# PixArt-alpha/PixArt-sigma

Measured on AMD Instinct MI355X. Metric: denoising steps/sec (fwd+bwd) PixArt-Sigma-XL/2 1024px bs16 @1/2/4/8 GPU, higher is better.
Workload: dtype fp16; 1 GPU; PixArt-Sigma-XL/2 1024px training step (fwd+bwd+clip+AdamW), batch 16/GPU, L=300 text tokens, DP=1 RCCL all-reduce; model=PixArtMS_XL_2, global_batch=16, seq_len=4096, parallelism=dp1, grad_checkpoint=False, optimizer=adamw, text_lens=all 300

## Files before the change

### pixart_sigma_amd/csrc/gemm.hip

```cpp
#include <atomic>
#include "common.h"
#include "gemm_params.h"
#include "../../include/pixart_hip.h"
#include <cstdio>
#include <cstdlib>
#include <cstring>

namespace {
using namespace pxa;

constexpr int BM = 128, BN = 128, BK = 64;
constexpr int KC_BYTES = 128 * BK * 2;
constexpr int RC_STRIDE = (128 + 32) * 2;
constexpr int RC_BYTES = BK * RC_STRIDE;


template <bool KC>
__device__ __forceinline__ void g2r(const bf16_t* __restrict__ X, int ld, int r0, int R, int k0, int kend, uint4 (&reg)[4], int tid) {
#pragma unroll
  for (int i = 0; i < 4; i++) {
    const bf16_t* src;
    bool ok;
    if (KC) {
      int c = tid & 7, row = (tid >> 3) + 32 * i;
// ... 566 lines not shown
    return frag_p<true, 256, 32>(lds, rbase, ks, lane);
  } else {
    const int gg = lane >> 4, tt = lane & 15, hi2 = gg >> 1;
    const int kr = ks * 16 + 8 * hi2 + (tt >> 2), col = rbase + 16 * (gg & 1) + (tt & 3) * 4;
    const int blk = col >> 5, inblk = (col & 31) * 2;
    const char* p0 = lds + (kr << (rows_log2 + 1)) + ((blk ^ (kr & 3)) << 6) + inblk;
    const char* p1 = lds + ((kr + 4) << (rows_log2 + 1)) + ((blk ^ ((kr + 4) & 3)) << 6) + inblk;
    return concat_tr(lds_tr_read(p0), lds_tr_read(p1));
  }
}

__device__ __forceinline__ bf16x8 frag16_kc(const char* lds, int rbase, int lane) {
  const int row = rbase + (lane & 15);
  return *reinterpret_cast<const bf16x8*>(lds + row * 64 + (((lane >> 4) ^ kc_swz<true>(row)) << 4));
}
template <bool KC>
__device__ __forceinline__ bf16x8 frag16(const char* lds, int rbase, int lane, int rows_log2) {
  if constexpr (KC) {
    return frag16_kc(lds, rbase, lane);
  } else {
    const int gg = lane >> 4, tt = lane & 15;
    const int kr = 8 * gg + (tt >> 2), col = rbase + (tt & 3) * 4;
    const int blk = col >> 5, inblk = ((col & 31) * 2) ^ ((gg & 1) << 5);
    const char* p0 = lds + (kr << (rows_log2 + 1)) + ((blk ^ (kr & 3)) << 6) + inblk;
    const char* p1 = lds + ((kr + 4) << (rows_log2 + 1)) + ((blk ^ ((kr + 4) & 3)) << 6) + inblk;
    return concat_tr(lds_tr_read(p0), lds_tr_read(p1));
  }
}

#ifndef GEMM_TRACE
#define GEMM_TRACE 0
#endif
#if GEMM_TRACE
__device__ unsigned long long g_trace[12][8];
#define PXA_TR(k) do { if (blockIdx.x == 8 && tid == 0 && tr_i < 12) g_trace[tr_i][k] = __builtin_readcyclecounter(); } while (0)
#else
#define PXA_TR(k) do {} while (0)
#endif
__device__ unsigned g_sched[64][16];
__device__ unsigned g_sched_word[64][512];

template <int LAYOUT, int EPI, int RM, bool SEG = false>
__global__ __launch_bounds__(512) void gemm_pers_kernel(GemmParams p) {
  constexpr bool A_KC = (LAYOUT != 2), B_KC = (LAYOUT == 0);
  constexpr int NW = 8, TM = 4, TN = 2, BKT = 32, H1 = 2;
  constexpr bool PH16 = GEMM_PHASE16 < 0 ? (LAYOUT != 0) : (GEMM_PHASE16 != 0);
  constexpr bool M16 = ((GEMM_M16 >> LAYOUT) & 1) && !(GEMM_ABL & 4);
  constexpr int UNIT = 40960;
  extern __shared__ __attribute__((aligned(16))) char smem[];
  const int tid = threadIdx.x, lane = tid & 63, wave = __builtin_amdgcn_readfirstlane(tid >> 6), wm = wave >> 2, wn = wave & 3, hi = lane >> 5;
  const bool late = wave >= NW / 2;
  char* stg = smem + 3 * UNIT + wave * 4096;
  const int mt = (p.M + 255) / 256, ntf = p.N / 256, remn = p.N - ntf * 256;
  constexpr bool PAIR = (RM == 1), HALF = (RM == 2);
  const bool remcol = RM != 0 && remn > 0 && remn <= 128;
  const int ntp = remcol ? ntf : (p.N + 255) / 256;
  const int rem_pg = remcol ? (PAIR ? 4 : 8) : 0;
  const int per_group = 8 * ntp + rem_pg, tiles = mt * ntp + (remcol ? (PAIR ? (mt + 1) / 2 : mt) : 0), T = tiles * p.split;
  auto units_of = [&](int z) { return (min(p.K, (z + 1) * p.k_per_split) - z * p.k_per_split) / BKT; };

  int m0a = 0, m0b = 0, n0 = 0, z_ = 0;
  bool vt = false;
  const int xq = T / 8, xr = T % 8;
  auto xs = [&](int x) { return x * xq + min(x, xr); };
  auto xc = [&](int x) { return xq + (x < xr ? 1 : 0); };
  auto locate_g = [&](int Lg) {
    z_ = Lg / tiles;
    const int t = Lg - z_ * tiles;
    const int g = t / per_group, in_g = t - g * per_group, first_m = g * 8, gsz = min(mt - first_m, 8), nfull = gsz * ntp;
    if (in_g < nfull) { vt = false; m0a = (first_m + in_g % gsz) * 256; m0b = m0a; n0 = (in_g / gsz) * 256; }
    else if (PAIR) { vt = true; m0a = (first_m + 2 * (in_g - nfull)) * 256; m0b = m0a + 256; n0 = ntf * 256; }
    else if (HALF) { vt = true; m0a = (first_m + (in_g - nfull)) * 256; m0b = m0a; n0 = ntf * 256; }
  };
  const bool rev = LAYOUT != 2 && p.desc != 0;
  auto pos_of = [&](int x, int i) { return xs(x) + (rev ? xc(x) - 1 - i : i); };
  auto locate = [&](int L) { locate_g(pos_of(L % 8, L / 8)); };
  const bool DYN = p.sched_slot >= 0;
  const int myx = blockIdx.x % 8;
  unsigned* sched = g_sched[p.sched_slot & 63];
  unsigned* sched_lds = reinterpret_cast<unsigned*>(smem + 32768);
  unsigned* sched_glb = &g_sched_word[p.sched_slot & 63][blockIdx.x & 511];
  auto publish = [&](int v) {
    if (PAIR) { if (lane == 0) __hip_atomic_store(sched_glb, (unsigned)v, __ATOMIC_RELAXED, __HIP_MEMORY_SCOPE_AGENT); wait_vmcnt<0>(); }
    else { if (lane == 0) sched_lds[0] = (unsigned)v; asm volatile("s_waitcnt lgkmcnt(0)" ::: "memory"); }
  };
  auto receive = [&]() -> int {
    const unsigned v = PAIR ? __hip_atomic_load(sched_glb, __ATOMIC_RELAXED, __HIP_MEMORY_SCOPE_AGENT) : sched_lds[0];
    return __builtin_amdgcn_readfirstlane((int)v);
  };
  unsigned pend = 0u;
  int nxt = -1;
  auto fetch_issue = [&]() {
    if (wave == 0 && lane == 0) {
      unsigned* cur = &sched[myx];
      const unsigned one = 1u;
      asm volatile("global_atomic_add %0, %1, %2, off sc0" : "=v"(pend) : "v"(cur), "v"(one) : "memory");
    }
  };
  auto fetch_resolve = [&]() -> int {
    int res = -1;
    asm volatile("" : "+v"(pend));
    if (lane == 0) {
      if ((int)pend < xc(myx)) res = pos_of(myx, (int)pend);
      else
        for (int k = 1; k < 8 && res < 0; k++) {
          const int x2 = (myx + k) & 7;
          const unsigned i2 = atomicAdd(&sched[x2], 1u);
          if ((int)i2 < xc(x2)) res = pos_of(x2, (int)i2);
        }
    }
    return __builtin_amdgcn_readfirstlane(res);
  };
  int L = blockIdx.x;
#if GEMM_STAGGER
  if (LAYOUT != 2 && ((blockIdx.x >> 3) & 1)) {
    const unsigned long long t0 = __builtin_amdgcn_s_memrealtime();
    while (__builtin_amdgcn_s_memrealtime() - t0 < (unsigned long long)GEMM_STAGGER) __builtin_amdgcn_s_sleep(32);
  }
#endif
  if (DYN) {
    fetch_issue();
    wait_vmcnt<0>();
// ... 3 lines not shown
    __syncthreads();
    if (first < 0) {
      if (wave == 0 && lane == 0 && atomicAdd(&sched[8], 1u) == gridDim.x - 1)
        for (int k = 0; k < 9; k++) sched[k] = 0u;
      return;
    }
    locate_g(first);
    fetch_issue();
  } else {
    locate(L);
  }
  int nk = units_of(z_), nk_pf = nk;
  const bf16_t* pp[5];
  long st[5];
  int dof[5];
  const long stepA = A_KC ? BKT : (long)BKT * p.lda, stepB = B_KC ? BKT : (long)BKT * p.ldb;
  int s_lo = 0, s_hi = 0;
  bool vt_pf = false;
  int dma_count = 0;
  auto piece = [&](int i, int slot) {
    dma_count++;
    lds_dma16(pp[i], smem + slot * UNIT + dof[i]);
#if !(GEMM_ABL & 1)
    pp[i] += st[i];
#endif
  };
  int seg_left0 = 0, seg_left1 = 0;
  int tap_kx0 = 0, tap_ky0 = 0, tap_half0 = 0, tap_kx1 = 0, tap_ky1 = 0, tap_half1 = 0;
#define PXA_SEG_ADVANCE(seg_left, tap_kx, tap_ky, tap_half, pa, pb)                                                          \
  do {                                                                                                                       \
    if (p.k_tap) {                                             \
      if (tap_half) {                                                                                                        \
        long adj;                                                                                                            \
        if (tap_kx < 2) { adj = p.k_tap - 64; tap_kx++; }                                                                    \
        else if (tap_ky < 2) { adj = p.tap_s - 2L * p.k_tap - 64; tap_kx = 0; tap_ky++; }                                    \
        else { adj = -2L * p.tap_s - 2L * p.k_tap; tap_kx = 0; tap_ky = 0; }                                                 \
        pa += adj; pb += adj;                                                                                                \
      }                                                                                                                      \
      tap_half ^= 1;                                                                                                         \
    } else {                                                                                                                 \
      seg_left -= BKT;                                                                                                       \
      if (seg_left == 0) { pa += p.seg_jump; pb += p.seg_jump; seg_left = p.k_seg; }                                         \
    }                                                                                                                        \
  } while (0)
  auto issue_lo = [&]() __attribute__((always_inline)) {
#pragma unroll
    for (int i = 0; i < H1; i++) piece(i, s_lo);
    if (SEG) PXA_SEG_ADVANCE(seg_left0, tap_kx0, tap_ky0, tap_half0, pp[0], pp[1]);
    s_lo = (s_lo + 1) & 3;
  };
  auto issue_hi = [&]() __attribute__((always_inline)) {
    piece(2, s_hi);
    if (!(HALF && vt_pf)) piece(3, s_hi);
    if (PAIR && vt_pf) piece(4, s_hi);
    if (SEG && PAIR) { if (vt_pf) PXA_SEG_ADVANCE(seg_left1, tap_kx1, tap_ky1, tap_half1, pp[2], pp[3]); }
    s_hi = (s_hi + 1) & 3;
  };
#undef PXA_SEG_ADVANCE
  auto prefetch = [&]() __attribute__((always_inline)) {
    vt_pf = (RM != 0) && vt;
    const long k0 = (long)z_ * p.k_per_split;
    const bool vq = PAIR && vt, hq = HALF && vt;
    const int rla = vq ? 9 : 8, rlb = (vq || hq) ? 7 : 8;
    const int ln = opaque<LAYOUT == 1 || (EPI >= 2 && EPI != 7) || (GEMM_EPI_EARLY && RM == 2)>(lane);
#pragma unroll
    for (int i = 0; i < 5; i++) {
      const int id = wave + NW * i;
      const bool is_a = vq ? (i < 4) : (i < 2);
      const int pid = is_a ? id : (vq ? id - 32 : id - 16);
      if (vq || (hq ? i < 3 : i < 4)) {
        if (is_a) pp[i] = piece_ptr_rt<A_KC, M16>(p.A, p.lda, m0a, m0b, p.M, pid * 64 + ln, rla) + (A_KC ? k0 : k0 * p.lda);
        else pp[i] = piece_ptr_rt<B_KC, M16>(p.B, p.ldb, n0, n0, p.N, pid * 64 + ln, rlb) + (B_KC ? k0 : k0 * p.ldb);
      }
      st[i] = is_a ? stepA : stepB;
      dof[i] = (is_a ? 0 : (vq ? 32768 : 16384)) + pid * 1024;
    }
    s_lo = s_hi = 0;
    dma_count = 0;
    if (SEG) { seg_left0 = seg_left1 = p.k_seg; tap_kx0 = tap_kx1 = tap_ky0 = tap_ky1 = tap_half0 = tap_half1 = 0; }
    issue_lo(); issue_hi(); issue_lo(); issue_hi();
    if (nk_pf > 2) { issue_lo(); if (PH16) issue_hi(); }
  };
  prefetch();
  int tr_i = 0; (void)tr_i;
  int prev_stores = 0;

  while (true) {
    f32x16 acc[TM][TN];
    f32x4 acc4[2 * TM][2 * TN];
#pragma unroll
    for (int i = 0; i < TM; i++)
#pragma unroll
      for (int j = 0; j < TN; j++)
#pragma unroll
        for (int g = 0; g < 16; g++) acc[i][j][g] = 0.f;
#pragma unroll
    for (int i = 0; i < 2 * TM; i++)
#pragma unroll
      for (int j = 0; j < 2 * TN; j++) acc4[i][j] = f32x4{0.f, 0.f, 0.f, 0.f};
#if GEMM_ABL & 4
    f32x4 a4[TM][TN][4];
#pragma unroll
    for (int i = 0; i < TM; i++)
#pragma unroll
      for (int j = 0; j < TN; j++)
#pragma unroll
        for (int q = 0; q < 4; q++) a4[i][j][q] = f32x4{0.f, 0.f, 0.f, 0.f};
#endif
    const bool vtc = PAIR && vt, hfc = HALF && vt;
    const int a_rb = hfc ? (wave >> 1) * 64 : (vtc ? (wn >> 1) * 256 : 0) + wm * 128, b_rb = (vtc || hfc) ? (wn & 1) * 64 : wn * 64;
    const int rla = vtc ? 9 : 8, rlb = (vtc || hfc) ? 7 : 8, boff = vtc ? 32768 : 16384;
    const int mw = hfc ? m0a + a_rb : ((vtc && (wn >> 1)) ? m0b : m0a) + wm * 128, nw = n0 + b_rb;
    const int tm_eff = hfc ? 2 : TM;
    const int zw = z_;
    PXA_TR(0);
    if (GEMM_STORE_OVERLAP && LAYOUT != 2 && EPI != 3) {
      if (prev_stores == 40) wait_vmcnt<40>();
      else if (prev_stores == 36) wait_vmcnt<36>();
      else if (prev_stores == 32) wait_vmcnt<32>();
      else if (prev_stores == 28) wait_vmcnt<28>();
      else if (prev_stores == 24) wait_vmcnt<24>();
      else if (prev_stores == 20) wait_vmcnt<20>();
      else if (prev_stores == 16) wait_vmcnt<16>();
      else if (prev_stores == 12) wait_vmcnt<12>();
      else if (prev_stores == 8) wait_vmcnt<8>();
      else wait_vmcnt<0>();
    } else {
      wait_vmcnt<0>();
    }
    if (DYN && wave == 0) {
      publish(fetch_resolve());
    }
    __builtin_amdgcn_s_barrier();
    if (DYN) nxt = receive();
    if (late) __builtin_amdgcn_s_barrier();
    PXA_TR(1);
    constexpr bool EARLY = GEMM_EPI_EARLY && M16 && LAYOUT != 2;
    constexpr bool AUXA = EARLY && (EPI == 2 || EPI == 4 || EPI == 6) && !(GEMM_ABL & 16);
    typedef unsigned u32x2 __attribute__((ext_vector_type(2)));
    u32x2 axa[2][2][4];
    f32x4 bq[2 * TN];
    const bool has_bias = EARLY && p.bias != nullptr;
    auto bias_issue = [&]() {
      const int R4b = lane >> 4;
#pragma unroll
      for (int jn = 0; jn < 2 * TN; jn++) {
        const float* src = p.bias + min(nw + jn * 16 + 4 * R4b, p.N - 4);
        asm volatile("global_load_dwordx4 %0, %1, off" : "=v"(bq[jn]) : "v"(src) : "memory");
      }
    };
    auto aux_issue = [&](int i, u32x2 (&dst)[2][4]) {
      const int R4a = lane >> 4, c16a = lane & 15;
#pragma unroll
      for (int mh = 0; mh < 2; mh++)
#pragma unroll
        for (int jn = 0; jn < 4; jn++) {
          const int m = min(mw + i * 32 + 16 * mh + c16a, p.M - 1), n = min(nw + jn * 16 + 4 * R4a, p.N - 4);
          const bf16_t* src = p.aux + (size_t)m * p.ldaux + n;
          asm volatile("global_load_dwordx2 %0, %1, off" : "=v"(dst[mh][jn]) : "v"(src) : "memory");
        }
    };
    auto unit16 = [&](int t, auto rem_c, auto th_c) {
// ... 131 lines not shown
#pragma unroll
    for (int i = 0; i < TM; i++)
#pragma unroll
      for (int j = 0; j < TN; j++)
#pragma unroll
        for (int g = 0; g < 16; g++) acc[i][j][g] = a4[i][j][g >> 2][g & 3];
#endif
    PXA_TR(2);
    if constexpr (LAYOUT != 2) {
      if (has_bias) bias_issue();
      if constexpr (AUXA) { aux_issue(0, axa[0]); aux_issue(1, axa[1]); }
    }
    if (!late) __builtin_amdgcn_s_barrier();
    PXA_TR(3);

    bool more = false;
    int pf_ops = 0;
    auto hand_over = [&]() {
      if (DYN) {
        more = nxt >= 0;
        if (more) {
          locate_g(nxt);
          nk_pf = units_of(z_);
          prefetch();
          fetch_issue();
        }
      } else {
        L += gridDim.x;
        more = L < T;
        if (more) {
          locate(L);
          nk_pf = units_of(z_);
          prefetch();
        }
      }
      if (more) pf_ops = dma_count;
    };
    const int le = opaque<LAYOUT == 1 || (EPI >= 2 && EPI != 7) || (GEMM_EPI_EARLY && RM == 2)>(lane);
    const int srow = le & 31;
    if constexpr (LAYOUT == 2) {
      hand_over();
      PXA_TR(4);
#pragma unroll
      for (int i = 0; i < TM; i++)
#pragma unroll
        for (int j = 0; j < TN; j++) {
          if constexpr (M16) {
#pragma unroll
            for (int mh = 0; mh < 2; mh++)
#pragma unroll
              for (int nh = 0; nh < 2; nh++) {
                const f32x4 a = acc4[2 * i + mh][2 * j + nh];
                const int row = 16 * mh + (lane & 15);
                *reinterpret_cast<float4*>(stg + row * 128 + (((4 * nh + (lane >> 4)) ^ (row & 7)) << 4)) = make_float4(a[0], a[1], a[2], a[3]);
              }
          } else {
#pragma unroll
          for (int q = 0; q < 4; q++)
            *reinterpret_cast<float4*>(stg + srow * 128 + (((q * 2 + hi) ^ (srow & 7)) << 4)) =
                make_float4(acc[i][j][q * 4], acc[i][j][q * 4 + 1], acc[i][j][q * 4 + 2], acc[i][j][q * 4 + 3]);
          }
          __builtin_amdgcn_s_waitcnt(0xc07f);
#pragma unroll
          for (int t4 = 0; t4 < 4; t4++) {
            const int row = t4 * 8 + (lane >> 3), ch = lane & 7;
            float4 v = *reinterpret_cast<const float4*>(stg + row * 128 + ((ch ^ (row & 7)) << 4));
            const int mm = mw + i * 32 + row, nn = nw + j * 32 + ch * 4;
            if (mm < p.M && nn < p.N) {
              if (p.accumulate == 3) {
                *reinterpret_cast<float4*>(p.slab + ((size_t)zw * p.M + mm) * p.N + nn) = v;
              } else {
                float* dst = p.outf + (size_t)mm * p.ldf + nn;
                if (p.accumulate) { const float4 o = *reinterpret_cast<const float4*>(dst); v.x += o.x; v.y += o.y; v.z += o.z; v.w += o.w; }
                *reinterpret_cast<float4*>(dst) = v;
              }
            }
          }
          __builtin_amdgcn_s_waitcnt(0xc07f);
        }
      nk = nk_pf;
      if (!more) break;
      continue;
    }
    const int act = (EPI == 0 || EPI == 5) ? 0 : EPI == 1 ? 3 : EPI == 2 ? 4 : (EPI == 4 || EPI == 6) ? 5 : EPI == 7 ? 1 : p.act;
    constexpr bool want_st = (EPI == 5 || EPI == 6);
    const bool dual = EPI == 1 || (EPI == 3 && ((p.act == 1 && p.out2 != nullptr) || p.act == 3));
    const bool want_cs = !(GEMM_ABL & 8) && (EPI == 2 || (EPI == 3 && p.colsum != nullptr));
    auto bias_apply = [&]() {
      asm volatile("" : "+v"(bq[0]), "+v"(bq[1]), "+v"(bq[2]), "+v"(bq[3]));
#pragma unroll
      for (int jn = 0; jn < 2 * TN; jn++)
#pragma unroll
        for (int mt = 0; mt < 2 * TM; mt++) acc4[mt][jn] += bq[jn];
    };
    auto bias_add = [&]() {
      const int R4b = le >> 4;
      if constexpr (M16) {
#pragma unroll
        for (int jn = 0; jn < 2 * TN; jn++) {
          const int n = nw + jn * 16 + 4 * R4b;
          const float4 b4 = (p.bias && n < p.N) ? *reinterpret_cast<const float4*>(p.bias + n) : make_float4(0.f, 0.f, 0.f, 0.f);
#pragma unroll
          for (int mt = 0; mt < 2 * TM; mt++) { acc4[mt][jn][0] += b4.x; acc4[mt][jn][1] += b4.y; acc4[mt][jn][2] += b4.z; acc4[mt][jn][3] += b4.w; }
        }
      } else {
#pragma unroll
        for (int j = 0; j < TN; j++)
#pragma unroll
          for (int q = 0; q < 4; q++) {
            const int n = nw + j * 32 + 8 * q + 4 * hi;
            const float4 b4 = (p.bias && n < p.N) ? *reinterpret_cast<const float4*>(p.bias + n) : make_float4(0.f, 0.f, 0.f, 0.f);
#pragma unroll
            for (int i = 0; i < TM; i++) { acc[i][j][q * 4] += b4.x; acc[i][j][q * 4 + 1] += b4.y; acc[i][j][q * 4 + 2] += b4.z; acc[i][j][q * 4 + 3] += b4.w; }
          }
      }
    };
    auto wait_allow = [&](int allowed) {
      if (allowed >= 28) wait_vmcnt<28>();
      else if (allowed >= 26) wait_vmcnt<26>();
      else if (allowed >= 24) wait_vmcnt<24>();
// ... 180 lines not shown
        }
      }
      static_assert(!(PAIR && (EPI == 2 || EPI == 3)), "column sums in a paired instance: guard their atomics with mw < p.M as the statistics are");
      if (want_cs) {
#pragma unroll
        for (int e = 0; e < 8; e++) {
          float v = cs[e];
          if (LPR <= 4) v += __shfl_xor(v, 4);
          v += __shfl_xor(v, 8); v += __shfl_xor(v, 16); v += __shfl_xor(v, 32);
          const int n = nw + j0 * 32 + (lane % LPR) * 8 + e;
          if (lane < LPR && n < p.N) atomicAdd(p.colsum + (size_t)((mw >> 7) % PXA_COLSUM_SLOTS) * p.colsum_stride + n, v);
        }
      }
      if (want_st && mw < p.M) {
        float* dst = p.gn_part + ((size_t)((mw >> 7) % PXA_COLSUM_SLOTS) * p.gn_B + st_img) * (p.N / 4) * 2;
#pragma unroll
        for (int h = 0; h < 2; h++) {
          float v = cs[h], u = sq[h];
          if (LPR <= 4) { v += __shfl_xor(v, 4); u += __shfl_xor(u, 4); }
          v += __shfl_xor(v, 8); v += __shfl_xor(v, 16); v += __shfl_xor(v, 32);
          u += __shfl_xor(u, 8); u += __shfl_xor(u, 16); u += __shfl_xor(u, 32);
          const int n = nw + j0 * 32 + (lane % LPR) * 8 + 4 * h;
          if (lane < LPR && n < p.N) { atomicAdd(dst + (n >> 2) * 2, v); atomicAdd(dst + (n >> 2) * 2 + 1, u); }
        }
      }
    };
    if (GEMM_ABL & 2) {
      float sacc = 0.f;
#pragma unroll
      for (int i = 0; i < TM; i++)
#pragma unroll
        for (int j = 0; j < TN; j++) sacc += acc[i][j][0] + acc[i][j][7] + acc[i][j][15];
      if (sacc == 123.456f) p.out[lane] = (bf16_t)sacc;
    } else {
#pragma unroll
      for (int j0 = 0; j0 + 1 < TN; j0 += 2) emit(j0, IntC<2>{});
      if constexpr (TN % 2 == 1) emit(TN - 1, IntC<1>{});
    }
    PXA_TR(5);
#if GEMM_TRACE
    tr_i++;
#endif
    {
      const bool interior = mw + tm_eff * 32 <= p.M && nw + 64 <= p.N;
      prev_stores = (interior && p.out && !(want_st && p.up_rp)) ? tm_eff * 4 * ((dual && !(GEMM_ABL & 32)) ? 2 : 1) + (want_st ? 4 : 0) + (want_cs ? 8 : 0) + ((AUXA && tm_eff > 2) ? 16 : 0) : 0;
    }
    nk = nk_pf;
    if (!more) break;
  }
  if (DYN && wave == 0 && lane == 0 && atomicAdd(&sched[8], 1u) == gridDim.x - 1)
    for (int k = 0; k < 9; k++) sched[k] = 0u;
}

struct GemmKnobs { bool no_staged, no_pers, no_half, seg_half; int tile; bool ascending, no_glds; };
GemmKnobs read_gemm_knobs() {
  static const bool no_staged = getenv("PXA_GEMM_NO_STAGED_EPILOGUE") != nullptr;
  static const bool no_pers = getenv("PXA_GEMM_NO_PERSISTENT") != nullptr;
  static const bool no_half = getenv("PXA_GEMM_NO_HALF_ITEMS") != nullptr;
  static const bool seg_half = getenv("PXA_GEMM_SEG_HALF") != nullptr;
  static const int tile = [] { const char* f = getenv("PXA_GEMM_TILE"); return f ? atoi(f) * (strstr(f, "x128") ? -1 : 1) : 0; }();
  static const bool ascending = getenv("PXA_GEMM_ASCENDING") != nullptr;
  return GemmKnobs{no_staged, no_pers, no_half, seg_half, tile, ascending, getenv("PXA_GEMM_NO_GLDS") != nullptr};
}
int dynamic_items_env() { return getenv("PXA_GEMM_STATIC") ? 0 : getenv("PXA_GEMM_DYNAMIC") ? 1 : -1; }
std::atomic<int> g_dynamic_items{-1}; std::atomic<unsigned> g_launch_seq{0};
bool dynamic_items() {
  int expect = -1;
  if (g_dynamic_items.load(std::memory_order_relaxed) < 0) g_dynamic_items.compare_exchange_strong(expect, dynamic_items_env() == 1 ? 1 : 0);
  return g_dynamic_items.load(std::memory_order_relaxed) != 0;
}
bool pers_halfcol(int N) { return N % 256 > 0 && N % 256 <= 128; }
int pers_tiles(int M, int N, int rm) {
  const int mt = (M + 255) / 256, ntf = N / 256;
  if (rm == 2 && pers_halfcol(N)) return mt * ntf + mt;
  const bool pairing = rm == 1 && pers_halfcol(N);
  return mt * (pairing ? ntf : (N + 255) / 256) + (pairing ? (mt + 1) / 2 : 0);
}
void cost_model(int M, int N, int K, int& split, int& tile) {
  struct Cfg { int tile, bm, bn, slots; double rate; };
  const Cfg cfgs[2] = {{128, 128, 128, 512, 760e12}, {256, 256, 256, 256, 1050e12}};
  double best = 1e30;
  for (const Cfg& c : cfgs) {
    if (c.tile == 256 && (M < 256 || N < 256)) continue;
    const long tiles = c.tile == 256 ? pers_tiles(M, N, 1) : (long)((M + c.bm - 1) / c.bm) * ((N + c.bn - 1) / c.bn);
    for (int sp = 1; sp <= 16; sp++) {
      const int kp = ((K + sp - 1) / sp + BK - 1) / BK * BK;
      if ((long)kp * (sp - 1) >= K) continue;
      const long rounds = (tiles * sp + c.slots - 1) / c.slots;
      const double t = rounds * (double)kp * c.bm * c.bn * 2.0 / (c.rate / c.slots) + (sp > 1 ? 2.0 * sp * M * N * 4.0 / 3.5e12 + 4e-6 : 0.0);
      if (t < best) { best = t; split = sp; tile = c.tile; }
    }
  }
}
int fill_gemm(const pxa_gemm_args* a, const GemmKnobs& k, GemmParams& p, int& tile) {
  PXA_CHECK(a && a->A && a->B, "pxa_gemm: null operand");
  PXA_CHECK(a->layout >= 0 && a->layout <= 2, "pxa_gemm: bad layout %d", a->layout);
  PXA_CHECK(a->M > 0 && a->N > 0 && a->K > 0, "pxa_gemm: bad shape %d %d %d", a->M, a->N, a->K);
  PXA_CHECK(a->N % 8 == 0, "pxa_gemm: N=%d must be a multiple of 8", a->N);
  PXA_CHECK(a->lda % 8 == 0 && a->ldb % 8 == 0, "pxa_gemm: lda/ldb must be multiples of 8 (16-byte rows)");
  if (a->layout != 2) PXA_CHECK(a->K % 8 == 0, "pxa_gemm: K=%d must be a multiple of 8 for k-contiguous A", a->K);
  if (a->layout == 2) PXA_CHECK(a->M % 8 == 0, "pxa_gemm: M=%d must be a multiple of 8 for layout TN", a->M);
  PXA_CHECK(a->out_bf16 || a->out_f32, "pxa_gemm: no output");
  if (a->out_bf16 || a->out2_bf16) PXA_CHECK(a->ld_out % 4 == 0, "pxa_gemm: ld_out must be a multiple of 4");
  if (a->out_f32) PXA_CHECK(a->ld_f32 % 4 == 0, "pxa_gemm: ld_f32 must be a multiple of 4");
  PXA_CHECK(a->act >= 0 && a->act <= 5, "pxa_gemm: bad act %d", a->act);
  if (a->act == 2 || a->act == 4 || a->act == 5) PXA_CHECK(a->aux && a->ldaux % 4 == 0, "pxa_gemm: act=%d needs aux", a->act);
  if (a->act == 3) PXA_CHECK(a->out_bf16 && a->out2_bf16, "pxa_gemm: act=3 needs both bf16 outputs");
  if (a->colsum) PXA_CHECK(a->out_bf16 && !a->out_f32, "pxa_gemm: colsum needs a bf16 output");
  int split = a->split_k < 1 ? 1 : a->split_k;
  if (split > 1) PXA_CHECK(a->out_f32 && a->accumulate && !a->out_bf16 && a->act == 0 && !a->bias, "pxa_gemm: split_k>1 needs fp32 atomic accumulate output only");
  p.A = (const bf16_t*)a->A; p.B = (const bf16_t*)a->B; p.lda = a->lda; p.ldb = a->ldb; p.M = a->M; p.N = a->N; p.K = a->K;
  p.bias = a->bias; p.aux = (const bf16_t*)a->aux; p.ldaux = a->ldaux; p.out = (bf16_t*)a->out_bf16; p.out2 = (bf16_t*)a->out2_bf16; p.ldo = a->ld_out;
  p.outf = a->out_f32; p.ldf = a->ld_f32; p.act = a->act; p.accumulate = a->accumulate; tile = 0;
  p.desc = (a->items_descending && !k.ascending) ? 1 : 0;
  p.k_seg = a->k_seg; p.seg_jump = a->k_seg ? a->a_seg_stride - a->k_seg : 0; p.k_tap = a->k_seg ? a->k_tap : 0; p.tap_s = a->a_seg_stride;
  if (a->k_seg && a->k_tap) PXA_CHECK(a->k_tap % BK == 0 && a->k_seg == 3 * a->k_tap && a->K == 3 * a->k_seg, "pxa_gemm: k_tap=%d needs k_seg = 3 k_tap, K = 9 k_tap, k_tap a multiple of %d", a->k_tap, BK);
  if (a->k_seg) {
    PXA_CHECK(a->layout == 0 && split == 1 && !a->colsum, "pxa_gemm: k_seg needs layout NT, no split-K, no colsum");
    PXA_CHECK(a->k_seg > 0 && a->k_seg % BK == 0 && a->K % a->k_seg == 0 && a->a_seg_stride % 8 == 0, "pxa_gemm: k_seg=%d must be a multiple of %d dividing K=%d (segment stride a multiple of 8)", a->k_seg, BK, a->K);
  }
  if (a->split_k == 0 && a->out_f32 && a->accumulate && !a->out_bf16 && a->act == 0 && !a->bias && a->K % BK == 0) cost_model(a->M, a->N, a->K, split, tile);
  p.k_per_split = ((a->K + split - 1) / split + BK - 1) / BK * BK;
  split = p.split = (a->K + p.k_per_split - 1) / p.k_per_split; p.tile_hint = tile; p.sched_slot = -1; p.slab = nullptr;
  p.colsum = a->colsum; p.colsum_stride = a->colsum_stride; p.gn_part = a->gn_part; p.gn_img_rows = a->gn_img_rows; p.gn_rp = a->gn_row_pitch; p.gn_h = a->gn_h; p.gn_w = a->gn_w;
  p.gn_B = 0; p.gn_inv_rp = 0.f; p.up_rp = 0; p.up_ip = 0; p.up_off = 0;
  if (a->up_row_pitch) {
    PXA_CHECK(a->gn_part && a->k_seg && a->act == 0 && !a->k_tap, "pxa_gemm: up_row_pitch needs an implicit convolution with gn_part, act 0 and the plain segment order");
    PXA_CHECK(a->K == 2 * a->k_seg && a->up_row_pitch == 2 * a->gn_w + 2 && a->up_img_rows >= (2 * a->gn_h + 2) * a->up_row_pitch && (a->up_dy | 1) == 1 && (a->up_dx | 1) == 1,
              "pxa_gemm: bad upsampled-convolution phase (K=%d k_seg=%d up_row_pitch=%d up_img_rows=%d dy=%d dx=%d)", a->K, a->k_seg, a->up_row_pitch, a->up_img_rows, a->up_dy, a->up_dx);
    PXA_CHECK(a->M >= 1024 && a->N % 128 == 0 && (long)(a->M / a->gn_img_rows) * a->up_img_rows < (1L << 31), "pxa_gemm: upsampled-convolution phase needs the persistent path (M >= 1024, N a multiple of 128)");
    p.up_rp = a->up_row_pitch; p.up_ip = a->up_img_rows; p.up_off = a->up_dy * a->up_row_pitch + a->up_dx;
  }
  if (a->gn_part) {
    PXA_CHECK(a->k_seg && a->out_bf16 && !a->out_f32 && (a->act == 0 || a->act == 5), "pxa_gemm: gn_part needs an implicit convolution (k_seg) with a bf16 output and act 0 or 5");
    PXA_CHECK(a->gn_img_rows > 0 && a->gn_img_rows % 256 == 0 && a->M % a->gn_img_rows == 0, "pxa_gemm: gn_img_rows=%d must be a multiple of 256 dividing M=%d", a->gn_img_rows, a->M);
    PXA_CHECK(a->gn_row_pitch == a->gn_w + 2 && a->gn_h > 0 && a->gn_w > 0 && (long)(a->gn_h + 2) * a->gn_row_pitch <= a->gn_img_rows && a->gn_img_rows < (1 << 22),
              "pxa_gemm: bad padded-grid geometry for gn_part (h=%d w=%d row_pitch=%d img_rows=%d)", a->gn_h, a->gn_w, a->gn_row_pitch, a->gn_img_rows);
    p.gn_B = a->M / a->gn_img_rows; p.gn_inv_rp = 1.0f / (float)a->gn_row_pitch;
  }
  if (p.accumulate && p.outf) {
    if (split == 1) p.accumulate = 2;
    else if (a->splitk_ws && a->splitk_ws_elems >= (long)split * a->M * a->N) { p.accumulate = 3; p.slab = a->splitk_ws; }
  }
  return 0;
}
enum class GemmFamily { simple, glds, pers };
enum GldsEpi { GLDS_DIRECT = 0, GLDS_STAGED = 1 };
enum PersEpi { PERS_PLAIN = 0, PERS_GELU_SAVE_GRAD = 1, PERS_MUL_AUX_COLSUM = 2, PERS_GENERIC = 3, PERS_ADD_AUX = 4, PERS_STATS = 5, PERS_ADD_AUX_STATS = 6, PERS_GELU = 7 };
struct GemmPlan {
  GemmFamily family; int layout, tile, epi, rm;
  bool seg; int split;
  bool try_nt4;
  bool colsum_pass_after;
};
int choose_gemm(const GemmParams& p, int layout, int split, int tile_hint, const GemmKnobs& k, GemmPlan& g) {
  g = GemmPlan{GemmFamily::simple, layout, 0, 0, 0, p.k_seg != 0, p.k_seg ? 1 : split, false, false};
  const bool bf16_only = p.out && !p.outf, hc = pers_halfcol(p.N);
  if (p.k_seg) {
    if (layout != 0) return -2;
    if (bf16_only && (p.act == 0 || p.act == 5) && p.M >= 1024 && p.N >= 128 && p.N % 128 == 0 && p.k_seg % 32 == 0 && !k.no_pers) {
      const bool pair = hc && !k.seg_half && p.M >= 512;
      g.family = GemmFamily::pers; g.rm = pair ? 1 : hc ? 2 : 0;
      g.epi = p.gn_part ? (p.act == 5 ? PERS_ADD_AUX_STATS : PERS_STATS) : (p.act == 5 ? PERS_ADD_AUX : PERS_PLAIN);
      return 0;
    }
    if (p.gn_part) { pxa_set_error("pxa_gemm: gn_part needs the persistent implicit-convolution path (bf16 output, M >= 1024, N a multiple of 128)"); return -1; }
    g.family = GemmFamily::glds; g.epi = bf16_only && p.act == 0 ? GLDS_STAGED : GLDS_DIRECT;
    return 0;
  }
  if (p.K % BK != 0 || p.k_per_split % BK != 0 || k.no_glds) { g.colsum_pass_after = p.colsum != nullptr; return 0; }
  const int want = k.tile ? k.tile : tile_hint ? tile_hint : (p.M >= 1024 && p.N >= 1024) ? 256 : 128, tile = want == 128 ? 0 : want == -256 ? 1 : 2;
  const bool pers_ok = tile == 2 && !k.no_pers;
  if (layout != 2 && pers_ok && split == 1 && bf16_only) {
    const bool half = hc && !k.no_half;
    g.family = GemmFamily::pers; g.try_nt4 = layout == 0 && p.act == 0 && !p.colsum;
    if (p.act == 0 && !p.colsum) { g.epi = PERS_PLAIN; g.rm = half ? 2 : 0; }
    else if (p.act == 3 && !p.colsum) g.epi = PERS_GELU_SAVE_GRAD;
    else if (p.act == 4 && p.colsum) { g.epi = PERS_MUL_AUX_COLSUM; g.rm = half ? 2 : 0; }
    else if (layout == 0 && p.act == 1 && !p.out2 && !p.colsum && !half) g.epi = PERS_GELU;
    else g.epi = PERS_GENERIC;
    return 0;
  }
  if (layout == 2 && pers_ok && p.outf && !p.out && !p.bias && p.act == 0 && p.accumulate != 1 && !p.colsum) { g.family = GemmFamily::pers; g.rm = hc ? 1 : 0; return 0; }
  const bool dual = (p.act == 1 && p.out2 != nullptr) || p.act == 3;
  g.family = GemmFamily::glds; g.tile = tile;
  g.epi = layout != 2 && bf16_only && !dual && !k.no_staged ? GLDS_STAGED : GLDS_DIRECT;
  g.colsum_pass_after = g.epi == GLDS_DIRECT && p.colsum != nullptr;
  return 0;
}
int plan_gemm(const pxa_gemm_args* a, GemmParams& p, GemmPlan& g) {
  const GemmKnobs k = read_gemm_knobs();
  int tile;
  const int rc = fill_gemm(a, k, p, tile);
  return rc ? rc : choose_gemm(p, a->layout, p.split, tile, k, g);
}

template <int LAYOUT, int EPI, int RM, bool SEG>
int launch_pers(GemmParams p, int split, hipStream_t s) {
  static_assert(!SEG || LAYOUT == 0, "segmented A: layout NT");
  p.split = split; constexpr int LDSP = 4 * 40960;
  hipError_t e = lds_optin(reinterpret_cast<const void*>(gemm_pers_kernel<LAYOUT, EPI, RM, SEG>), LDSP);
  if (e != hipSuccess) { pxa_set_error("hipFuncSetAttribute(gemm_pers<%d,%d>): %s", LAYOUT, EPI, hipGetErrorString(e)); return -3; }
  static int n_cu = 0;
  if (!n_cu) {
    int dev = 0; hipDeviceProp_t prop;
    if (hipGetDevice(&dev) != hipSuccess || hipGetDeviceProperties(&prop, dev) != hipSuccess) { pxa_set_error("gemm_pers: device query failed"); return -3; }
    n_cu = prop.multiProcessorCount;
  }
  const int tiles = pers_tiles(p.M, p.N, RM) * split;
  p.sched_slot = dynamic_items() ? (int)(g_launch_seq.fetch_add(1u) & 63u) : -1;
  hipLaunchKernelGGL((gemm_pers_kernel<LAYOUT, EPI, RM, SEG>), dim3(tiles < n_cu ? tiles : n_cu), dim3(512), LDSP, s, p);
  PXA_LAUNCH_CHECK(); return 0;
}
template <int LAYOUT, int TBM, int TBN, int WM, int WN, int EPI, bool SEG>
int launch_glds_e(GemmParams p, int split, hipStream_t s) {
  p.split = split; constexpr int LDSG = 2 * (TBM + TBN) * 128;
  static_assert(WM * WN * (TBM / WM) * EPI_STRIDE <= LDSG, "staged epilogue must fit the operand stages");
  hipError_t e = lds_optin(reinterpret_cast<const void*>(gemm_glds_kernel<LAYOUT, TBM, TBN, WM, WN, EPI, SEG>), LDSG);
  if (e != hipSuccess) { pxa_set_error("hipFuncSetAttribute(gemm_glds<%d,%d,%d>): %s", LAYOUT, TBM, TBN, hipGetErrorString(e)); return -3; }
  dim3 grid(((p.M + TBM - 1) / TBM) * ((p.N + TBN - 1) / TBN) * split, 1, 1);
  hipLaunchKernelGGL((gemm_glds_kernel<LAYOUT, TBM, TBN, WM, WN, EPI, SEG>), grid, dim3(WM * WN * 64), LDSG, s, p);
  PXA_LAUNCH_CHECK(); return 0;
}
template <int LAYOUT>
int launch_simple(GemmParams p, int split, hipStream_t s) {
  p.split = split; constexpr bool A_KC = (LAYOUT != 2), B_KC = (LAYOUT == 0);
  constexpr int LDS = 2 * ((A_KC ? KC_BYTES : RC_BYTES) + (B_KC ? KC_BYTES : RC_BYTES));
  hipError_t e = lds_optin(reinterpret_cast<const void*>(gemm_kernel<LAYOUT>), LDS);
  if (e != hipSuccess) { pxa_set_error("hipFuncSetAttribute(gemm<%d>, %d): %s", LAYOUT, LDS, hipGetErrorString(e)); return -3; }
  dim3 grid(((p.M + BM - 1) / BM) * ((p.N + BN - 1) / BN) * split, 1, 1);
  hipLaunchKernelGGL(gemm_kernel<LAYOUT>, grid, dim3(256), LDS, s, p);
  PXA_LAUNCH_CHECK(); return 0;
}
int launch_instance(const GemmPlan& g, GemmParams p, hipStream_t s) {
#define PXA_KEY(f, l, t, e, r, sg) ((((((int)(f) * 3 + (l)) * 3 + (t)) * 8 + (e)) * 3 + (r)) * 2 + ((sg) ? 1 : 0))
#define PXA_SIMPLE(L) case PXA_KEY(GemmFamily::simple, L, 0, 0, 0, false): return launch_simple<L>(p, g.split, s);
#define PXA_GLDS(L, T, TBM, TBN, WM, WN, E, SG) case PXA_KEY(GemmFamily::glds, L, T, E, 0, SG): return launch_glds_e<L, TBM, TBN, WM, WN, E, SG>(p, g.split, s);
#define PXA_GLDS3(L, E) PXA_GLDS(L, 0, 128, 128, 2, 2, E, false) PXA_GLDS(L, 1, 256, 128, 4, 2, E, false) PXA_GLDS(L, 2, 256, 256, 2, 4, E, false)
#define PXA_PERS(L, E, RM, SG) case PXA_KEY(GemmFamily::pers, L, 0, E, RM, SG): return launch_pers<L, E, RM, SG>(p, g.split, s);
#define PXA_TOKEN(L) PXA_PERS(L, PERS_PLAIN, 0, false) PXA_PERS(L, PERS_PLAIN, 2, false) PXA_PERS(L, PERS_GELU_SAVE_GRAD, 0, false) PXA_PERS(L, PERS_MUL_AUX_COLSUM, 0, false) PXA_PERS(L, PERS_MUL_AUX_COLSUM, 2, false) PXA_PERS(L, PERS_GENERIC, 0, false)
#define PXA_CONV(E) PXA_PERS(0, E, 0, true) PXA_PERS(0, E, 1, true) PXA_PERS(0, E, 2, true)
  if (g.colsum_pass_after) p.colsum = nullptr;
  switch (PXA_KEY(g.family, g.layout, g.tile, g.epi, g.rm, g.seg)) {
    PXA_SIMPLE(0) PXA_SIMPLE(1) PXA_SIMPLE(2) PXA_GLDS3(0, GLDS_DIRECT) PXA_GLDS3(0, GLDS_STAGED) PXA_GLDS3(1, GLDS_DIRECT) PXA_GLDS3(1, GLDS_STAGED)
    PXA_GLDS3(2, GLDS_DIRECT) PXA_GLDS3(2, GLDS_STAGED) PXA_GLDS(0, 0, 128, 128, 2, 2, GLDS_DIRECT, true) PXA_GLDS(0, 0, 128, 128, 2, 2, GLDS_STAGED, true) PXA_TOKEN(0) PXA_TOKEN(1)
    PXA_PERS(0, PERS_GELU, 0, false) PXA_PERS(2, PERS_PLAIN, 0, false) PXA_PERS(2, PERS_PLAIN, 1, false) PXA_CONV(PERS_PLAIN) PXA_CONV(PERS_ADD_AUX) PXA_CONV(PERS_STATS) PXA_CONV(PERS_ADD_AUX_STATS)
  }
  pxa_set_error("pxa_gemm: no kernel instance for the chosen plan"); return -2;
}

__global__ __launch_bounds__(256) void splitk_reduce_kernel(const float* __restrict__ slab, float* __restrict__ out, int ld, int M, int N, int split) {
  const long i4 = blockIdx.x * 256L + threadIdx.x, n4 = N / 4;
  if (i4 >= (long)M * n4) return;
  const int m = i4 / n4, n = (i4 - (long)m * n4) * 4;
  float4 s = *reinterpret_cast<const float4*>(out + (size_t)m * ld + n);
  for (int z = 0; z < split; z++) {
    const float4 v = *reinterpret_cast<const float4*>(slab + ((size_t)z * M + m) * N + n);
    s.x += v.x; s.y += v.y; s.z += v.z; s.w += v.w;
  }
  *reinterpret_cast<float4*>(out + (size_t)m * ld + n) = s;
}
}
// ... 48 lines not shown
```

### pixart_sigma_amd/csrc/gemm_params.h

```cpp
#pragma once
#include "common.h"

struct GemmParams {
  const bf16_t* A; const bf16_t* B; int lda, ldb;
  int M, N, K;
  const float* bias; const bf16_t* aux; int ldaux;
  bf16_t* out; bf16_t* out2; int ldo;
  float* outf; int ldf;
  int act, accumulate, k_per_split, tile_hint, split, sched_slot;
  int desc;
  float* slab;
  float* colsum;
  long colsum_stride;
  int k_seg;
  long seg_jump;
  int k_tap;
  long tap_s;
  float* gn_part; int gn_img_rows, gn_rp, gn_h, gn_w, gn_B; float gn_inv_rp;
  int up_rp, up_ip, up_off;
};

int pxa_gemm_nt4_launch(const GemmParams& p, hipStream_t stream);
```

Measured before the change: 2.381 steps/s.

## Pair transposed row-remainder tiles in persistent TN GEMM

For the TN layout (layout 2) with M leaving a half-tile row remainder, the persistent GEMM now handles the last partial row strip by swapping the roles of A and B. Pairs of N tiles are computed as a paired tile, and the staged epilogue writes the result transposed. This avoids padding the 128-row remainder up to a full 256-row tile, which wasted MFMA work and occupied slots in the persistent schedule. The cost is extra index logic, scalar transposed LDS stores in the epilogue, and forcing the PAIR path on for all layout-2 instantiations. An environment knob restores the old padding behaviour.

```diff
diff --git a/pixart_sigma_amd/csrc/gemm.hip b/pixart_sigma_amd/csrc/gemm.hip
--- a/pixart_sigma_amd/csrc/gemm.hip
+++ b/pixart_sigma_amd/csrc/gemm.hip
@@ -642,22 +642,32 @@
   const bool late = wave >= NW / 2;
   char* stg = smem + 3 * UNIT + wave * 4096;
   const int mt = (p.M + 255) / 256, ntf = p.N / 256, remn = p.N - ntf * 256;
-  constexpr bool PAIR = (RM == 1), HALF = (RM == 2);
+  constexpr bool PAIR = (RM == 1) || (LAYOUT == 2), HALF = (RM == 2);
   const bool remcol = RM != 0 && remn > 0 && remn <= 128;
   const int ntp = remcol ? ntf : (p.N + 255) / 256;
   const int rem_pg = remcol ? (PAIR ? 4 : 8) : 0;
-  const int per_group = 8 * ntp + rem_pg, tiles = mt * ntp + (remcol ? (PAIR ? (mt + 1) / 2 : mt) : 0), T = tiles * p.split;
+  const bool remrow = LAYOUT == 2 && p.tn_rowrem != 0;
+  const int mtF = remrow ? mt - 1 : mt, ntr = remrow ? (ntp + 1) / 2 : 0;
+  const int per_group = 8 * ntp + rem_pg, tiles_main = mtF * ntp + (remcol ? (PAIR ? (mt + 1) / 2 : mt) : 0), tiles = tiles_main + ntr, T = tiles * p.split;
   auto units_of = [&](int z) { return (min(p.K, (z + 1) * p.k_per_split) - z * p.k_per_split) / BKT; };
 
   int m0a = 0, m0b = 0, n0 = 0, z_ = 0;
-  bool vt = false;
+  bool vt = false, tr = false;
   const int xq = T / 8, xr = T % 8;
   auto xs = [&](int x) { return x * xq + min(x, xr); };
   auto xc = [&](int x) { return xq + (x < xr ? 1 : 0); };
   auto locate_g = [&](int Lg) {
     z_ = Lg / tiles;
     const int t = Lg - z_ * tiles;
-    const int g = t / per_group, in_g = t - g * per_group, first_m = g * 8, gsz = min(mt - first_m, 8), nfull = gsz * ntp;
+    if (LAYOUT == 2) {
+      tr = t >= tiles_main;
+      if (tr) {
+        const int c2 = 2 * (t - tiles_main);
+        vt = true; m0a = c2 * 256; m0b = c2 + 1 < ntp ? m0a + 256 : ((p.N + 255) / 256) * 256; n0 = mtF * 256;
+        return;
+      }
+    }
+    const int g = t / per_group, in_g = t - g * per_group, first_m = g * 8, gsz = min(mtF - first_m, 8), nfull = gsz * ntp;
     if (in_g < nfull) { vt = false; m0a = (first_m + in_g % gsz) * 256; m0b = m0a; n0 = (in_g / gsz) * 256; }
     else if (PAIR) { vt = true; m0a = (first_m + 2 * (in_g - nfull)) * 256; m0b = m0a + 256; n0 = ntf * 256; }
     else if (HALF) { vt = true; m0a = (first_m + (in_g - nfull)) * 256; m0b = m0a; n0 = ntf * 256; }
@@ -767,27 +777,30 @@
   auto issue_hi = [&]() __attribute__((always_inline)) {
     piece(2, s_hi);
     if (!(HALF && vt_pf)) piece(3, s_hi);
-    if (PAIR && vt_pf) piece(4, s_hi);
+    if (PAIR && (LAYOUT == 2 ? __builtin_expect(vt_pf, true) : vt_pf)) piece(4, s_hi);
     if (SEG && PAIR) { if (vt_pf) PXA_SEG_ADVANCE(seg_left1, tap_kx1, tap_ky1, tap_half1, pp[2], pp[3]); }
     s_hi = (s_hi + 1) & 3;
   };
 #undef PXA_SEG_ADVANCE
   auto prefetch = [&]() __attribute__((always_inline)) {
-    vt_pf = (RM != 0) && vt;
+    vt_pf = (PAIR || HALF) && vt;
     const long k0 = (long)z_ * p.k_per_split;
     const bool vq = PAIR && vt, hq = HALF && vt;
     const int rla = vq ? 9 : 8, rlb = (vq || hq) ? 7 : 8;
     const int ln = opaque<LAYOUT == 1 || (EPI >= 2 && EPI != 7) || (GEMM_EPI_EARLY && RM == 2)>(lane);
+    const bool tq = LAYOUT == 2 && tr;
+    const bf16_t* const Xa = tq ? p.B : p.A; const bf16_t* const Xb = tq ? p.A : p.B;
+    const int ld_a = tq ? p.ldb : p.lda, ld_b = tq ? p.lda : p.ldb, R_a = tq ? p.N : p.M, R_b = tq ? p.M : p.N;
 #pragma unroll
     for (int i = 0; i < 5; i++) {
       const int id = wave + NW * i;
       const bool is_a = vq ? (i < 4) : (i < 2);
       const int pid = is_a ? id : (vq ? id - 32 : id - 16);
       if (vq || (hq ? i < 3 : i < 4)) {
-        if (is_a) pp[i] = piece_ptr_rt<A_KC, M16>(p.A, p.lda, m0a, m0b, p.M, pid * 64 + ln, rla) + (A_KC ? k0 : k0 * p.lda);
-        else pp[i] = piece_ptr_rt<B_KC, M16>(p.B, p.ldb, n0, n0, p.N, pid * 64 + ln, rlb) + (B_KC ? k0 : k0 * p.ldb);
-      }
-      st[i] = is_a ? stepA : stepB;
+        if (is_a) pp[i] = piece_ptr_rt<A_KC, M16>(Xa, ld_a, m0a, m0b, R_a, pid * 64 + ln, rla) + (A_KC ? k0 : k0 * ld_a);
+        else pp[i] = piece_ptr_rt<B_KC, M16>(Xb, ld_b, n0, n0, R_b, pid * 64 + ln, rlb) + (B_KC ? k0 : k0 * ld_b);
+      }
+      st[i] = (is_a != tq) ? stepA : stepB;
       dof[i] = (is_a ? 0 : (vq ? 32768 : 16384)) + pid * 1024;
     }
     s_lo = s_hi = 0;
@@ -822,7 +835,7 @@
 #pragma unroll
         for (int q = 0; q < 4; q++) a4[i][j][q] = f32x4{0.f, 0.f, 0.f, 0.f};
 #endif
-    const bool vtc = PAIR && vt, hfc = HALF && vt;
+    const bool vtc = PAIR && vt, hfc = HALF && vt, trc = LAYOUT == 2 && tr;
     const int a_rb = hfc ? (wave >> 1) * 64 : (vtc ? (wn >> 1) * 256 : 0) + wm * 128, b_rb = (vtc || hfc) ? (wn & 1) * 64 : wn * 64;
     const int rla = vtc ? 9 : 8, rlb = (vtc || hfc) ? 7 : 8, boff = vtc ? 32768 : 16384;
     const int mw = hfc ? m0a + a_rb : ((vtc && (wn >> 1)) ? m0b : m0a) + wm * 128, nw = n0 + b_rb;
@@ -1060,11 +1073,25 @@
               for (int nh = 0; nh < 2; nh++) {
                 const f32x4 a = acc4[2 * i + mh][2 * j + nh];
                 const int row = 16 * mh + (lane & 15);
+                if (trc) {
+#pragma unroll
+                  for (int g = 0; g < 4; g++) {
+                    const int c = 16 * nh + 4 * (lane >> 4) + g;
+                    *reinterpret_cast<float*>(stg + c * 128 + (((row >> 2) ^ (c & 7)) << 4) + (row & 3) * 4) = a[g];
+                  }
+                } else
                 *reinterpret_cast<float4*>(stg + row * 128 + (((4 * nh + (lane >> 4)) ^ (row & 7)) << 4)) = make_float4(a[0], a[1], a[2], a[3]);
               }
           } else {
 #pragma unroll
           for (int q = 0; q < 4; q++)
+            if (trc) {
+#pragma unroll
+              for (int g = 0; g < 4; g++) {
+                const int c = 8 * q + 4 * hi + g;
+                *reinterpret_cast<float*>(stg + c * 128 + (((srow >> 2) ^ (c & 7)) << 4) + (srow & 3) * 4) = acc[i][j][q * 4 + g];
+              }
+            } else
             *reinterpret_cast<float4*>(stg + srow * 128 + (((q * 2 + hi) ^ (srow & 7)) << 4)) =
                 make_float4(acc[i][j][q * 4], acc[i][j][q * 4 + 1], acc[i][j][q * 4 + 2], acc[i][j][q * 4 + 3]);
           }
@@ -1073,7 +1100,7 @@
           for (int t4 = 0; t4 < 4; t4++) {
             const int row = t4 * 8 + (lane >> 3), ch = lane & 7;
             float4 v = *reinterpret_cast<const float4*>(stg + row * 128 + ((ch ^ (row & 7)) << 4));
-            const int mm = mw + i * 32 + row, nn = nw + j * 32 + ch * 4;
+            const int mm = trc ? nw + j * 32 + row : mw + i * 32 + row, nn = trc ? mw + i * 32 + ch * 4 : nw + j * 32 + ch * 4;
             if (mm < p.M && nn < p.N) {
               if (p.accumulate == 3) {
                 *reinterpret_cast<float4*>(p.slab + ((size_t)zw * p.M + mm) * p.N + nn) = v;
@@ -1360,7 +1387,7 @@
     for (int k = 0; k < 9; k++) sched[k] = 0u;
 }
 
-struct GemmKnobs { bool no_staged, no_pers, no_half, seg_half; int tile; bool ascending, no_glds; };
+struct GemmKnobs { bool no_staged, no_pers, no_half, seg_half; int tile; bool ascending, tn_pad_rows, no_glds; };
 GemmKnobs read_gemm_knobs() {
   static const bool no_staged = getenv("PXA_GEMM_NO_STAGED_EPILOGUE") != nullptr;
   static const bool no_pers = getenv("PXA_GEMM_NO_PERSISTENT") != nullptr;
@@ -1368,7 +1395,8 @@
   static const bool seg_half = getenv("PXA_GEMM_SEG_HALF") != nullptr;
   static const int tile = [] { const char* f = getenv("PXA_GEMM_TILE"); return f ? atoi(f) * (strstr(f, "x128") ? -1 : 1) : 0; }();
   static const bool ascending = getenv("PXA_GEMM_ASCENDING") != nullptr;
-  return GemmKnobs{no_staged, no_pers, no_half, seg_half, tile, ascending, getenv("PXA_GEMM_NO_GLDS") != nullptr};
+  static const bool tn_pad_rows = getenv("PXA_GEMM_TN_PAD_ROWS") != nullptr;
+  return GemmKnobs{no_staged, no_pers, no_half, seg_half, tile, ascending, tn_pad_rows, getenv("PXA_GEMM_NO_GLDS") != nullptr};
 }
 int dynamic_items_env() { return getenv("PXA_GEMM_STATIC") ? 0 : getenv("PXA_GEMM_DYNAMIC") ? 1 : -1; }
 std::atomic<int> g_dynamic_items{-1}; std::atomic<unsigned> g_launch_seq{0};
@@ -1378,19 +1406,21 @@
   return g_dynamic_items.load(std::memory_order_relaxed) != 0;
 }
 bool pers_halfcol(int N) { return N % 256 > 0 && N % 256 <= 128; }
-int pers_tiles(int M, int N, int rm) {
+bool pers_rowrem(int layout, int M, const GemmKnobs& k) { return layout == 2 && M >= 256 && pers_halfcol(M) && !k.tn_pad_rows; }
+int pers_tiles(int M, int N, int rm, bool rowrem) {
   const int mt = (M + 255) / 256, ntf = N / 256;
   if (rm == 2 && pers_halfcol(N)) return mt * ntf + mt;
   const bool pairing = rm == 1 && pers_halfcol(N);
-  return mt * (pairing ? ntf : (N + 255) / 256) + (pairing ? (mt + 1) / 2 : 0);
-}
-void cost_model(int M, int N, int K, int& split, int& tile) {
+  const int ntp = pairing ? ntf : (N + 255) / 256;
+  return (rowrem ? mt - 1 : mt) * ntp + (pairing ? (mt + 1) / 2 : 0) + (rowrem ? (ntp + 1) / 2 : 0);
+}
+void cost_model(int M, int N, int K, bool rowrem, int& split, int& tile) {
   struct Cfg { int tile, bm, bn, slots; double rate; };
   const Cfg cfgs[2] = {{128, 128, 128, 512, 760e12}, {256, 256, 256, 256, 1050e12}};
   double best = 1e30;
   for (const Cfg& c : cfgs) {
     if (c.tile == 256 && (M < 256 || N < 256)) continue;
-    const long tiles = c.tile == 256 ? pers_tiles(M, N, 1) : (long)((M + c.bm - 1) / c.bm) * ((N + c.bn - 1) / c.bn);
+    const long tiles = c.tile == 256 ? pers_tiles(M, N, 1, rowrem) : (long)((M + c.bm - 1) / c.bm) * ((N + c.bn - 1) / c.bn);
     for (int sp = 1; sp <= 16; sp++) {
       const int kp = ((K + sp - 1) / sp + BK - 1) / BK * BK;
       if ((long)kp * (sp - 1) >= K) continue;
@@ -1427,7 +1457,8 @@
     PXA_CHECK(a->layout == 0 && split == 1 && !a->colsum, "pxa_gemm: k_seg needs layout NT, no split-K, no colsum");
     PXA_CHECK(a->k_seg > 0 && a->k_seg % BK == 0 && a->K % a->k_seg == 0 && a->a_seg_stride % 8 == 0, "pxa_gemm: k_seg=%d must be a multiple of %d dividing K=%d (segment stride a multiple of 8)", a->k_seg, BK, a->K);
   }
-  if (a->split_k == 0 && a->out_f32 && a->accumulate && !a->out_bf16 && a->act == 0 && !a->bias && a->K % BK == 0) cost_model(a->M, a->N, a->K, split, tile);
+  p.tn_rowrem = pers_rowrem(a->layout, a->M, k) ? 1 : 0;
+  if (a->split_k == 0 && a->out_f32 && a->accumulate && !a->out_bf16 && a->act == 0 && !a->bias && a->K % BK == 0) cost_model(a->M, a->N, a->K, p.tn_rowrem != 0, split, tile);
   p.k_per_split = ((a->K + split - 1) / split + BK - 1) / BK * BK;
   split = p.split = (a->K + p.k_per_split - 1) / p.k_per_split; p.tile_hint = tile; p.sched_slot = -1; p.slab = nullptr;
   p.colsum = a->colsum; p.colsum_stride = a->colsum_stride; p.gn_part = a->gn_part; p.gn_img_rows = a->gn_img_rows; p.gn_rp = a->gn_row_pitch; p.gn_h = a->gn_h; p.gn_w = a->gn_w;
@@ -1515,7 +1546,7 @@
     if (hipGetDevice(&dev) != hipSuccess || hipGetDeviceProperties(&prop, dev) != hipSuccess) { pxa_set_error("gemm_pers: device query failed"); return -3; }
     n_cu = prop.multiProcessorCount;
   }
-  const int tiles = pers_tiles(p.M, p.N, RM) * split;
+  const int tiles = pers_tiles(p.M, p.N, RM, LAYOUT == 2 && p.tn_rowrem) * split;
   p.sched_slot = dynamic_items() ? (int)(g_launch_seq.fetch_add(1u) & 63u) : -1;
   hipLaunchKernelGGL((gemm_pers_kernel<LAYOUT, EPI, RM, SEG>), dim3(tiles < n_cu ? tiles : n_cu), dim3(512), LDSP, s, p);
   PXA_LAUNCH_CHECK(); return 0;
diff --git a/pixart_sigma_amd/csrc/gemm_params.h b/pixart_sigma_amd/csrc/gemm_params.h
--- a/pixart_sigma_amd/csrc/gemm_params.h
+++ b/pixart_sigma_amd/csrc/gemm_params.h
@@ -18,6 +18,7 @@
   long tap_s;
   float* gn_part; int gn_img_rows, gn_rp, gn_h, gn_w, gn_B; float gn_inv_rp;
   int up_rp, up_ip, up_off;
+  int tn_rowrem;
 };
 
 int pxa_gemm_nt4_launch(const GemmParams& p, hipStream_t stream);
```

Result: no change. 2.378 steps/s (-0.1%).
